# Rinoahu/SwiftOrtho

Measured on AMD Instinct MI355X. Metric: M query-aa/s scanned all-vs-all, higher is better.
Workload: dtype u8/int16/int32 (5-bit packed residues, packed 16-bit score-only DP, int32 traced DP); 1 GPU; BASELINE config 3: 100000 synthetic proteins x 300 aa self-search, seed 11111011111, aa9, -M 120000000, -c 50000 (2 chunks), -e 1e-5, -v 500; query_aa=30007201, rows=1618760

## Files before the change

swiftortho_amd/csrc/host.h:

```cpp
#pragma once
#include "common.h"
#include "kernels.h"
#include "seedhash.h"
#include "../../include/sohit.h"

#include <algorithm>
#include <array>
#include <atomic>
#include <chrono>
#include <cmath>
#include <cstring>
#include <functional>
#include <map>
#include <malloc.h>
#include <memory>
#include <mutex>
#include <thread>
#include <unordered_map>
#include <sys/stat.h>

inline double wall() { return std::chrono::duration<double>(std::chrono::steady_clock::now().time_since_epoch()).count(); }

extern double (*volatile p_pow)(double, double);
extern double (*volatile p_log)(double);
// ... 269 lines not shown
    u32 nq = 0;
    std::vector<u8> h_res;
    std::vector<u32> h_off;
    u32 maxqlen = 0;
    std::vector<u32> qid;
    std::vector<u8> qcls;
    u64 lay_gen = 0;
    i64 lay_lo = -1, lay_hi = -1;
    bool lay_classes = false;
    bool permuted = false;
    bool cls_sorted = true;
    u32 cls_start[QCLASSES_MAX + 1] = {0};
    u32 cls_maxq[QCLASSES_MAX] = {0};
    std::vector<u32> blkmax;
    u32 q_defer = 0;
    bool korder_async = false;
    bool korder_ready = false;
    u32 ksc_long = 0;
    DevBuf<u32> open_list;
    u32 n_open = 0;
    DevBuf<u8> kord_have;
    bool kord_have_clear = false;
    DevBuf<u32> d_qid, d_ocnt, d_ostart;
    SeqSet dev;
    DevBuf<u32> qbucket, korder, sbeg, scnt, pcnt, eff, nz, hoff, cidx;
    DevBuf<u32> sbeg2, scnt2, pcnt2;
    int bnd_ci = -1;
    DevBuf<int> ksc;
    DevBuf<u8> mark;
    DevBuf<u32> cs_hoff, cs_beg, blk_first, qseg, sel_idx;
    DevBuf<unsigned long long> qhits;
    DevBuf<u64> cs_kbase;
    DevBuf<u64> keys, keys2;
    DevBuf<u32> hits32, hits32s, bmat, bpart, bt0, btd, bext, bflag, bcnt, bccnt;
    DevBuf<u64> mlist;
    DevBuf<u32> flags, gidx, ghead;
    DevBuf<u64> p_qs, p_sd, p_ft, p_qs2, tmp64, q_qs, q_sd, q_ft;
    DevBuf<u32> shard;
    DevBuf<unsigned long long> stepshard;
    DevBuf<u32> pidx, pidx2, shead;
    DevBuf<u64> c_ft, c_ft2;
    DevBuf<u32> c_q, c_rec, order, order2;
    DevBuf<u32> counters;
    DevBuf<unsigned long long> ucount;
    DevBuf<u32> cand_q, cand_rec;
    std::vector<u32> chunk_base;
    DevBuf<u32> ccnt;
    DevBuf<unsigned long long> qcells;
    DevBuf<u32> tpos, spcnt, spoff, sidx, spec_trace, sel_a, sel_b;
    DevBuf<u64> gx;
    DevBuf<u32> gL, gR;
    DevBuf<u32> segfirst, st_state, rcnt, tcnt, roff, ridx, ridx2, ntile, roffc, rk_slot, order_tmp;
    DevBuf<u32> cqoff, prior, qtot, qcoff, fin_rec, perm, ntask, toff, sel, nout, ooff;
    DevBuf<AlnTask> tasks;
    DevBuf<AlnRes> ares;
    DevBuf<int> bits, outrec;
    DevBuf<u32> trace;
    DevBuf<u32> tr_units, tr_ofs;
    DevBuf<u32> tl_sorted, al_sorted;
    AlnChain aln;
};

#define QCLASSES 5
static_assert(QCLASSES <= QCLASSES_MAX, "Batch::cls_start");
inline u8 query_class(u32 len) { return len < 512 ? 0 : len < 1024 ? 1 : len < 2048 ? 2 : len < 4096 ? 3 : 4; }

// ... 278 lines not shown
```

swiftortho_amd/csrc/host_seed.hip:

```cpp
#include "host.h"

static void defer_long_class(so_ctx* c, Batch& b, u32 q_long) {
    b.korder_async = q_long < b.nq && b.cls_sorted && b.qcls[q_long] != b.qcls[0];
    if (!b.korder_async) return;
    b.q_defer = q_long;
    while (b.q_defer > 0 && b.qcls[b.q_defer - 1] == b.qcls[q_long]) --b.q_defer;
    HIP_CHECK(hipEventRecord(c->ev_side_go, c->st));
    HIP_CHECK(hipStreamWaitEvent(c->st_side, c->ev_side_go, 0));
}

void order_queries(so_ctx* c, Batch& b) {
    const u32 q_long = b.ksc_long;
    const size_t nres = b.h_off[b.nq];
    if (q_long < b.nq) b.gx.ensure(nres + 4), b.gL.ensure(nres + 4), b.gR.ensure(nres + 4);
    defer_long_class(c, b, q_long);
    launch_ksc_order(b.dev.d_scls.p, b.dev.d_off.p, b.nq, q_long, c->cfg.mink, c->d_b62c.p, b.gx.p, b.gL.p, b.gR.p, b.korder.p, c->st,
                     b.korder_async ? c->st_side : c->st);
    if (b.korder_async) HIP_CHECK(hipEventRecord(c->ev_korder, c->st_side));
    b.korder_ready = true;
}

void order_open_queries(so_ctx* c, Batch& b, const unsigned long long* qh) {
    u32 q_long = b.nq;
    for (u32 q = b.ksc_long; q < b.nq && q_long == b.nq; ++q)
// ... 531 lines not shown
                          c->ref.d_ug_store.p + U1_UG_PAD, c->ref.d_off.p + ch.seq_lo, c->d_b62c.p, b.bflag.p + 1, b.shard.p, b.p_qs.p, b.p_sd.p, b.p_ft.p, b.stepshard.p,
                          ug2 ? b.mlist.p : nullptr, b.bflag.p + 3, ugstat, c->st);
        if (ug2)
            launch_ungap2(c->ncu, b.mlist.p, b.bflag.p + 3, b.hits32s.p, b.bext.p, L, kl, klr, btab, U1_WAIT, b.dev.d_ug_store.p + U1_UG_PAD, b.dev.d_off.p,
                          c->ref.d_ug_store.p + U1_UG_PAD, c->ref.d_off.p + ch.seq_lo, c->d_b62c.p, b.bflag.p + 2, b.shard.p, b.p_qs.p, b.p_sd.p, b.p_ft.p, b.stepshard.p,
                          ugstat, c->st);
        else
            launch_ungap(w32 ? nullptr : b.keys2.p, Hv, kl, klr, btab, pmaxq >= gallop_min, ft_walk, b.dev.d_scls.p, b.dev.d_off.p, c->ref.d_scls4.p,
                         c->ref.d_off.p + ch.seq_lo, c->d_b62c.p, b.shard.p, shard_cap, b.p_qs.p, b.p_sd.p, b.p_ft.p, b.stepshard.p, c->st, w32 ? b.hits32s.p : nullptr,
                         b.bext.p, nb, &L, ug1, ugstat);
        bL = L;
        bL.R = (u32)(((u64)nseq_chunk + (1ull << wb) - 1) >> wb);
        bnb = bL.R * nqp;
        c->cnt.hits_bucketed += H;
        return true;
    };

    auto group_sorted = [&] {
    b.keys.ensure((size_t)H + 2), b.keys2.ensure((size_t)H + 2);
    const u32 nseg = qb - qa;
    const bool uq = tune().ungapq && tune().segsort && AS == 1 && compact && !ft_walk && UG_SHARDS == 1 && pmaxq <= ungapq_qcap() && nseg >= 256;
    if (uq || nseg >= 256) {
        b.qseg.ensure((size_t)b.nq + 4);
        launch_query_segments(b.hoff.p, b.dev.d_off.p, qa, qb, AS, H, b.qseg.p, c->st);
    }
    if (uq) {
        if (!c->ref.ug_valid) {
            const size_t nres = c->ref.res.size();
            c->ref.d_ug_store.ensure(nres + 2 * (size_t)U1_UG_PAD);
            launch_make_ug(c->ref.d_scls.p, c->ref.d_off.p, (u32)c->ref.N, nres, 8u, c->ref.d_ug_store.p + U1_UG_PAD, c->st);
            c->ref.ug_valid = true;
        }
        b.blk_first.ensure((size_t)nseg + 4), b.flags.ensure((size_t)nseg + 4);
        ProfTimer pt(c, &c->cnt.lookup_ms, &c->cnt.lookup_launches);
        launch_ungapq(c->ncu, b.qseg.p + qa, nseg, qa, b.blk_first.p, b.cs_hoff.p, b.cs_beg.p, b.cs_kbase.p, K, dk32, kl, klr, btab, b.dev.d_scls.p, b.dev.d_off.p,
                      c->ref.d_ug_store.p + U1_UG_PAD, c->ref.d_off.p + ch.seq_lo, c->d_b62c.p, b.bflag.p + 1, b.shard.p, b.p_qs.p, b.p_sd.p, b.p_ft.p, b.stepshard.p,
                      b.keys.p, b.keys2.p, b.flags.p, ugstat, c->st);
        pt.stop();
        if (c->profile) c->cnt.lookup_bytes += (i64)8 * (i64)H;
    } else {
    b.blk_first.ensure((size_t)lookup_num_blocks(H) + 2);
    launch_lookup_blockfirst(b.cs_hoff.p, K, H, b.blk_first.p, c->st);
    {
        ProfTimer pt(c, &c->cnt.lookup_ms, &c->cnt.lookup_launches);
        launch_lookup(b.cs_hoff.p, b.cs_beg.p, b.cs_kbase.p, b.blk_first.p, K, H, compact ? (const void*)dk32 : (const void*)ch.dkeys.p,
                      compact, c->ref.d_off.p + ch.seq_lo, kl, ch.maxslen, b.keys.p, c->st);
        pt.stop();
        if (c->profile) c->cnt.lookup_bytes += (i64)8 * (i64)H;
    }
    }
    t1 = wall();
    sc.lap("seed.compact_lookup");
    const int seg_mode = (int)tune().segsort;
    if (seg_mode && nseg >= 256) {
        ensure_sort_tmp(c, sort_keys_u64_seg_temp_bytes(H, nseg, kl.sh_diag, kl.sh_q));
        if (uq) sort_keys_u64_seg2(c->d_sort_tmp.p, c->d_sort_tmp.cap, b.keys.p, b.keys2.p, H, nseg, b.qseg.p + qa, b.flags.p, kl.sh_diag, kl.sh_q, c->st);
        else sort_keys_u64_seg(c->d_sort_tmp.p, c->d_sort_tmp.cap, b.keys.p, b.keys2.p, H, nseg, b.qseg.p + qa, kl.sh_diag, kl.sh_q, c->st);
    } else {
    ensure_sort_tmp(c, sort_keys_u64_temp_bytes(H, kl.total));
    sort_keys_u64(c->d_sort_tmp.p, c->d_sort_tmp.cap, b.keys.p, b.keys2.p, H, kl.sh_diag, kl.total, c->st);
    }
    sc.lap("group.sort_keys");
    launch_ungap(b.keys2.p, H, kl, klr, btab, pmaxq >= gallop_min, ft_walk, b.dev.d_scls.p, b.dev.d_off.p, c->ref.d_scls4.p, c->ref.d_off.p + ch.seq_lo,
                 c->d_b62c.p, b.shard.p, shard_cap, b.p_qs.p, b.p_sd.p, b.p_ft.p, b.stepshard.p, c->st, nullptr, nullptr, 0, nullptr, false, ugstat);
    };

    reset_pass_lists();
    if (!group_bucketed()) {
        bbest = false;
        group_sorted();
// ... 183 lines not shown
```

swiftortho_amd/csrc/k_ungapq.hip:

```cpp
#include "ungap1.h"

#define UQ_WAVES 16
#define UQ_RING 128
#define UQ_TBITS 12
#define UQ_QCAP 512
#define UQ_QSLOT (UQ_QCAP + 2 * U1_QPAD)
#define UQ_TILE 256
#define UQ_WAVE_BYTES (UQ_QSLOT + (1 << UQ_TBITS) / 4 + UQ_RING * 4 + UQ_RING * 4 + UQ_RING * 2 + UQ_TILE * 8)

__device__ __forceinline__ u32 bk_scan_max16(u32 x) {
    x = max(x, (u32)__builtin_amdgcn_update_dpp(0, (int)x, 0x111, 0xf, 0xf, true));
    x = max(x, (u32)__builtin_amdgcn_update_dpp(0, (int)x, 0x112, 0xf, 0xf, true));
    x = max(x, (u32)__builtin_amdgcn_update_dpp(0, (int)x, 0x114, 0xf, 0xf, true));
    x = max(x, (u32)__builtin_amdgcn_update_dpp(0, (int)x, 0x118, 0xf, 0xf, true));
    x = max(x, (u32)__builtin_amdgcn_update_dpp(0, (int)x, 0x142, 0xa, 0xf, false));
    x = max(x, (u32)__builtin_amdgcn_update_dpp(0, (int)x, 0x143, 0xc, 0xf, false));
    return x;
}

__device__ __forceinline__ u32 uq_slot(u32 g) { return (g * 2654435761u) >> (32 - UQ_TBITS); }

__global__ __launch_bounds__(256) void k_uq_first(const u32* __restrict__ qseg, u32 nqp, const u32* __restrict__ cs_hoff, u32 K, u32* __restrict__ qk) {
    const u32 q = blockIdx.x * 256u + threadIdx.x;
    if (q > nqp) return;
    const u32 x = qseg[q];
    u32 lo = 0, hi = K;
    while (lo < hi) {
        const u32 m = (lo + hi) >> 1;
        if (cs_hoff[m] < x) lo = m + 1;
        else hi = m;
    }
    qk[q] = lo;
}

template <bool BANDS, bool COUNT>
__global__ __launch_bounds__(64 * UQ_WAVES, 1) __attribute__((amdgpu_num_sgpr(96))) void k_ungapq(
    const u32* __restrict__ qseg , u32 nqp, u32 qa, const u32* __restrict__ qk, const u32* __restrict__ cs_hoff,
    const u32* __restrict__ cs_base, const u64* __restrict__ cs_kbase, const u32* __restrict__ dk32, int bp, int bd, int sh_q, int sh_qpos, int sh_diag, int diag_off, int rbs,
    int rsh_subj, int rsh_diag, int rdoff, const uint2* __restrict__ btab, u32 wait_n, const u8* __restrict__ q_scls, const u32* __restrict__ qoff,
    const u8* __restrict__ r_ug, const u32* __restrict__ roff, const signed char* __restrict__ b62g, u32* __restrict__ work_ctr, u32* __restrict__ shard_cnt,
    u64* __restrict__ p_qs, u64* __restrict__ p_sd, u64* __restrict__ p_ft, unsigned long long* __restrict__ group_count, u64* __restrict__ keys,
    u64* __restrict__ keys_sorted, u32* __restrict__ seg_end, unsigned long long* __restrict__ stat ) {
    constexpr int TSH = 3;
    constexpr u32 TBYTES = (u32)U1_ROWS << (8 + TSH);
    __shared__ __align__(16) unsigned char uq_smem[TBYTES + UQ_WAVES * UQ_WAVE_BYTES];
    const int lane = threadIdx.x & 63, w = threadIdx.x >> 6;
    for (u32 i = threadIdx.x; i < U1_ROWS * 32u * 32u; i += 64 * UQ_WAVES) {
        const u32 q = i >> 10, s = (i >> 5) & 31u, l = i & 31u;
        const int v = (q < SCLS_N && s < SCLS_N) ? (int)b62g[q * SCLS_N + s] : -100;
        *reinterpret_cast<short*>(uq_smem + ((q << 11) | (s << 6) | (l << 1))) = (short)v;
    }
    __syncthreads();
    unsigned char* wbase = uq_smem + TBYTES + (u32)w * UQ_WAVE_BYTES;
    u8* qslot = wbase;
    u32* tab = reinterpret_cast<u32*>(wbase + UQ_QSLOT);
    u32* ring_s = tab + (1 << UQ_TBITS) / 16;
    u32* ring_g = ring_s + UQ_RING;
    u16* ring_q = reinterpret_cast<u16*>(ring_g + UQ_RING);
    u32* mbase = reinterpret_cast<u32*>(ring_q + UQ_RING);
    u16* marks = reinterpret_cast<u16*>(mbase + UQ_TILE);
    u16* mqpos = marks + UQ_TILE;
    static_assert(UQ_TILE == 256, "tile_marks clears the marks with two words per lane");
    static_assert(U1_PCAP * 8 <= 7 * 64 && UQ_WAVES <= U1_ROWS, "pass buffer in a table row's tail");
    u64* s_pass = reinterpret_cast<u64*>(uq_smem + ((u32)w << 11) + 25 * 64);
    u16* s_passq = reinterpret_cast<u16*>(uq_smem + ((u32)w << 11) + 25 * 64 + U1_PCAP * 8);
    static_assert(U1_PCAP * 8 + U1_PCAP * 2 <= 7 * 64, "row tail");
    const unsigned long long lt = (1ull << lane) - 1ull;
    const u32 lanebase = (u32)(size_t)(__attribute__((address_space(3))) unsigned char*)uq_smem + ((u32)(lane & 31) << 1);
    const u32 pmask = (1u << bp) - 1u;
    const u32 dmask = (1u << bd) - 1u;
    u32 npb = 0, ngroups = 0;
    u32 ch_pos = 0, ch_end = 0;
    U1Track tr_unused;
    U1Count ct;
    ct.n = 0;
    ct.start();

    for (;;) {
        u32 qrel = 0;
        if (lane == 0) qrel = atomicAdd(work_ctr, 1u);
        qrel = (u32)__builtin_amdgcn_readfirstlane((int)qrel);
        if (qrel >= nqp) break;
        const u32 h0 = (u32)__builtin_amdgcn_readfirstlane((int)qseg[qrel]), h1 = (u32)__builtin_amdgcn_readfirstlane((int)qseg[qrel + 1]);
        if (h0 == h1) {
            if (lane == 0) seg_end[qrel] = h0;
            continue;
        }
        const u32 k0 = (u32)__builtin_amdgcn_readfirstlane((int)qk[qrel]), k1 = (u32)__builtin_amdgcn_readfirstlane((int)qk[qrel + 1]);
        const u32 gq = qa + qrel;
        const u32 qb0 = (u32)__builtin_amdgcn_readfirstlane((int)qoff[gq]);
        const int ql = (int)((u32)__builtin_amdgcn_readfirstlane((int)qoff[gq + 1]) - qb0);
        for (int i = lane * 16; i < UQ_QSLOT; i += 64 * 16) {
            const int p0 = i - U1_QPAD;
            uint4 v = make_uint4(0x18181818u, 0x18181818u, 0x18181818u, 0x18181818u);
            if (p0 >= 0 && p0 < ql) {
                v = u1_load16(q_scls + qb0 + (u32)p0);
                u32* d = reinterpret_cast<u32*>(&v);
#pragma unroll
                for (int k = 0; k < 4; ++k) {
                    const int nv = min(max(ql - p0 - 4 * k, 0), 4);
                    const u32 m = nv >= 4 ? 0xFFFFFFFFu : ((1u << (8 * nv)) - 1u);
                    d[k] = (d[k] & m) | (0x18181818u & ~m);
                }
                if (p0 == 0) d[0] = (d[0] & 0xFFFFFF00u) | 0x18u;
            }
            *reinterpret_cast<uint4*>(qslot + i) = v;
        }
        reinterpret_cast<uint4*>(tab)[lane] = make_uint4(0, 0, 0, 0);
        u1_wave_sync();
        const int qr_max = U1_QPAD + ql;
        const u64 kq = (u64)gq << sh_q;

        const u32 n = h1 - h0;
        u32 t_next = k0;
        u32 c_base = 0, c_qpos = 0;
        auto tile_marks = [&](u32 tb) {
            reinterpret_cast<u32*>(marks)[lane] = 0, reinterpret_cast<u32*>(marks)[64 + lane] = 0;
            u1_wave_sync();
            for (;;) {
                const u32 k = t_next + (u32)lane;
                u32 o = 0xFFFFFFFFu;
                if (k < k1) o = cs_hoff[k] - h0 - tb;
                const bool in = o < (u32)UQ_TILE;
                if (in) {
                    marks[o] = (u16)(o + 1u);
                    mbase[o] = cs_base[k] + h0;
                    mqpos[o] = (u16)((u32)(cs_kbase[k] >> sh_qpos) & pmask);
                }
                const u32 cnt = (u32)__popcll(__ballot(in));
                t_next += cnt;
                if (cnt < 64u) break;
            }
            u1_wave_sync();
        };
        auto gen_step = [&](u32 tb, u32 st, u32& c, u32& qpos, u32& o) -> bool {
            o = tb + 64u * st + (u32)lane;
            const u32 p1 = bk_scan_max16((u32)marks[64u * st + (u32)lane]);
            u32 base = c_base;
            qpos = c_qpos;
            if (p1) base = mbase[p1 - 1u], qpos = (u32)mqpos[p1 - 1u];
            c_base = (u32)__builtin_amdgcn_readlane((int)base, 63), c_qpos = (u32)__builtin_amdgcn_readlane((int)qpos, 63);
            c = 0xFFFFFFFFu;
            if (o >= n) return false;
            c = dk32[base + o];
            return (int)c >= 0;
        };
        for (u32 tb = 0; tb < n; tb += UQ_TILE) {
            tile_marks(tb);
            const u32 nst = (min(n - tb, (u32)UQ_TILE) + 63u) / 64u;
            for (u32 st = 0; st < nst; ++st) {
                u32 c, qpos, o;
                if (gen_step(tb, st, c, qpos, o)) {
                    const u32 t = uq_slot(c + qpos), sh = (t & 15u) * 2u;
                    const u32 old = atomicOr(&tab[t >> 4], 1u << sh);
                    if ((old >> sh) & 1u) atomicOr(&tab[t >> 4], 2u << sh);
                }
            }
        }
        u1_wave_sync();

        auto flush = [&]() {
            const u32 at = u1_reserve(npb, lane, ch_pos, ch_end, &shard_cnt[0], U1_CHUNK);
            if ((u32)lane < npb) {
                const u64 e = s_pass[lane];
                const u32 G = (u32)e, qp = (u32)s_passq[lane];
                u32 gsubj;
                int dlt;
                if (BANDS) {
                    const uint2 be = btab[G >> bd];
                    gsubj = be.x;
                    dlt = (int)(be.y - G);
                } else {
                    gsubj = G >> bd;
                    dlt = diag_off - (int)(G & dmask);
                }
                p_qs[at] = ((u64)gq << rbs) | gsubj;
                p_sd[at] = (e & 0xFFFFFFFF00000000ull) | (u64)(u32)dlt;
                p_ft[at] = ((u64)gsubj << rsh_subj) | ((u64)(u32)(rdoff - dlt) << rsh_diag) | ((u64)qp << sh_qpos);
            }
            npb = 0;
        };
        t_next = k0, c_base = 0, c_qpos = 0;
        u32 g_tb = 0, g_st = 0, g_nst = (min(n, (u32)UQ_TILE) + 63u) / 64u;
        tile_marks(0);
        bool more = true;
        u32 ns = 0;
        u32 rfront = 0, rback = 0;
        bool working = false;
        int qR = 0, qL = 0;
        i64 sR = 0, sL = 0;
        u32 hG = 0, hq = 0;
        pk16 S = {0, 0}, M = {0, 0};
        for (;;) {
            const unsigned long long idleb = __ballot(!working);
            if (idleb && ((u32)__popcll(idleb) >= wait_n || idleb == ~0ull)) {
                while (rback - rfront <= UQ_RING - 64u && more) {
                    u32 c, qpos, o;
                    const bool valid = gen_step(g_tb, g_st, c, qpos, o);
                    bool sing = false;
                    u32 G = 0;
                    if (valid) {
                        G = c + qpos;
                        const u32 t = uq_slot(G);
                        sing = ((tab[t >> 4] >> ((t & 15u) * 2u)) & 3u) == 1u;
                    }
                    const unsigned long long sb_ = __ballot(sing), kb_ = __ballot(valid && !sing);
                    if (valid && !sing) keys[h0 + ns + (u32)__popcll(kb_ & lt)] = kq + ((u64)qpos << sh_diag) + ((u64)qpos << sh_qpos) + ((u64)c << sh_diag);
                    ns += (u32)__popcll(kb_);
                    if (sing) {
                        u32 gsubj;
                        int dlt;
                        if (BANDS) {
                            const uint2 be = btab[G >> bd];
                            gsubj = be.x;
                            dlt = (int)(be.y - G);
                        } else {
                            gsubj = G >> bd;
                            dlt = diag_off - (int)(G & dmask);
                        }
                        const u32 slot = (rback + (u32)__popcll(sb_ & lt)) & (UQ_RING - 1);
                        ring_s[slot] = roff[gsubj] + (u32)((int)qpos + dlt);
                        ring_g[slot] = G;
                        ring_q[slot] = (u16)qpos;
                    }
                    rback += (u32)__popcll(sb_);
                    if (++g_st >= g_nst) {
                        g_st = 0, g_tb += UQ_TILE;
                        if (g_tb < n) {
                            g_nst = (min(n - g_tb, (u32)UQ_TILE) + 63u) / 64u;
                            tile_marks(g_tb);
                        } else {
                            more = false;
                        }
                    }
                }
                u1_wave_sync();
                const u32 avail = rback - rfront;
                if (!working) {
                    const u32 rk = (u32)__popcll(idleb & lt);
                    if (rk < avail) {
                        const u32 slot = (rfront + rk) & (UQ_RING - 1);
                        const u32 sa = ring_s[slot];
                        hG = ring_g[slot], hq = (u32)ring_q[slot];
                        qR = U1_QPAD + (int)hq, qL = qR - 16;
                        sR = (i64)sa, sL = (i64)sa - 16;
                        S = pk16{0, 0}, M = pk16{0, 0};
                        if (COUNT) ct.start();
                        working = true;
                    }
                }
                const u32 taken = min((u32)__popcll(idleb), avail);
                rfront += taken;
                ngroups += taken;
                u1_wave_sync();
            }
            if (!__ballot(working)) {
                if (!more && rback == rfront) break;
                continue;
            }
            bool fin = false;
            if (working) {
                const uint4 qr4 = u1_lds16(qslot, qR), ql4 = u1_lds16(qslot, qL);
                const uint4 sr4 = u1_load16(r_ug + sR), sl4 = u1_load16(r_ug + sL);
                const u32 msk = u1_step<TSH, false, COUNT>(qr4, ql4, sr4, sl4, lanebase, S, M, tr_unused, 0, ct);
                qR = min(qR + 16, qr_max), qL = max(qL - 16, 0);
                sR += 16, sL -= 16;
                fin = msk == 0xFFFFFFFFu;
            }
            {
                const int score = (int)M.x + (int)M.y;
                bool todo = fin && score >= MIN_UNGAP;
                for (;;) {
                    const unsigned long long pb = __ballot(todo);
                    if (!pb) break;
                    const u32 room = U1_PCAP - npb, rk = (u32)__popcll(pb & lt);
                    if (todo && rk < room) {
                        s_pass[npb + rk] = ((u64)(u32)score << 32) | hG;
                        s_passq[npb + rk] = (u16)hq;
                        todo = false;
                    }
                    npb += min((u32)__popcll(pb), room);
                    u1_wave_sync();
                    if (npb == U1_PCAP) {
                        flush();
                        u1_wave_sync();
                    }
                }
                if (fin) working = false;
            }
        }
        if (npb) {
            flush();
            u1_wave_sync();
        }
        if (lane == 0) seg_end[qrel] = h0 + ns;
        for (u32 i = h0 + ns + (u32)lane; i < h1; i += 64) keys_sorted[i] = ~0ull;
    }
    for (u32 i = ch_pos + (u32)lane; i < ch_end; i += 64) p_qs[i] = UG_REC_NONE, p_ft[i] = 0;
    if (lane == 0 && ngroups) atomicAdd(&group_count[0], (unsigned long long)ngroups);
    if (COUNT) {
        unsigned long long nst = ct.n;
#pragma unroll
        for (int o = 32; o > 0; o >>= 1) nst += __shfl_xor(nst, o);
        if (lane == 0) atomicAdd(&stat[0], nst), atomicAdd(&stat[1], (unsigned long long)ngroups);
    }
}

u32 ungapq_qcap() { return UQ_QCAP; }

void launch_ungapq(u32 ncu, const u32* qseg, u32 nqp, u32 qa, u32* qk, const u32* cs_hoff, const u32* cs_base, const u64* cs_kbase, u32 K, const u32* dk32,
                   const KeyLayout& kl, const KeyLayout& klr, const void* btab, const u8* q_scls, const u32* qoff, const u8* r_ug, const u32* roff, const signed char* b62g,
                   u32* work_ctr, u32* shard_cnt, u64* p_qs, u64* p_sd, u64* p_ft, unsigned long long* group_count, u64* keys, u64* keys_sorted, u32* seg_end,
                   unsigned long long* stat, hipStream_t st) {
    if (!nqp) return;
    hipLaunchKernelGGL(k_uq_first, dim3((nqp + 1 + 255) / 256), dim3(256), 0, st, qseg, nqp, cs_hoff, K, qk);
    static_assert(((size_t)U1_ROWS << 11) + (size_t)UQ_WAVES * UQ_WAVE_BYTES <= 160 * 1024, "LDS of a CU");
    const dim3 g(std::min<u32>(ncu, (nqp + UQ_WAVES - 1) / UQ_WAVES)), bl(64 * UQ_WAVES);
#define UQ_GO(B, CT)                                                                                                                                              \
    hipLaunchKernelGGL((k_ungapq<B, CT>), g, bl, 0, st, qseg, nqp, qa, qk, cs_hoff, cs_base, cs_kbase, dk32, kl.bp, kl.bd, kl.sh_q, kl.sh_qpos, kl.sh_diag, (int)kl.diag_off, klr.bs,  \
                       klr.sh_subj, klr.sh_diag, (int)klr.diag_off, (const uint2*)btab, U1_WAIT, q_scls, qoff, r_ug, roff, b62g, work_ctr, shard_cnt, p_qs, p_sd, p_ft,      \
                       group_count, keys, keys_sorted, seg_end, stat)
    if (stat) {
        if (btab) UQ_GO(true, true);
        else UQ_GO(false, true);
    } else if (btab) UQ_GO(true, false);
    else UQ_GO(false, false);
#undef UQ_GO
}
```

swiftortho_amd/csrc/kernels.h:

```cpp
#pragma once
#include "common.h"

struct HashLut;

size_t scan_u32_temp_elems(size_t n);
size_t effscan_temp_elems(size_t n);
const u32* effscan(const u8* mark, const u32* scnt, size_t n, u32* hoff, u32* cidx, u32* temp, hipStream_t st);
const u32* scan_u32(const u32* in, u32* out, size_t n, bool inclusive, u32* temp, hipStream_t st);
void fill_u32(u32* p, size_t n, u32 v, hipStream_t st);

size_t sort_keys_u64_temp_bytes(size_t n, int bits);
void sort_keys_u64(void* temp, size_t temp_bytes, const u64* in, u64* out, size_t n, int begin_bit, int end_bit, hipStream_t st);
void launch_query_segments(const u32* hoff, const u32* qoff, u32 qa, u32 qb, int AS, u32 H, u32* seg, hipStream_t st);
size_t sort_keys_u64_seg_temp_bytes(size_t n, u32 nseg, int begin_bit, int end_bit);
void sort_keys_u64_seg(void* temp, size_t temp_bytes, const u64* in, u64* out, size_t n, u32 nseg, const u32* seg, int begin_bit,
                       int end_bit, hipStream_t st);
void sort_keys_u64_seg2(void* temp, size_t temp_bytes, const u64* in, u64* out, size_t n, u32 nseg, const u32* seg_begin, const u32* seg_end, int begin_bit,
                        int end_bit, hipStream_t st);
void launch_stride_gather(const u32* src, u32 stride, u32 n, u32* dst, hipStream_t st);
size_t sort_pairs_u64_u32_temp_bytes(size_t n, int bits);
void sort_pairs_u64_u32(void* temp, size_t temp_bytes, const u64* kin, u64* kout, const u32* vin, u32* vout, size_t n, int bits,
                        hipStream_t st);
size_t sort_pairs_u64_u64_temp_bytes(size_t n, int bits);
void sort_pairs_u64_u64(void* temp, size_t temp_bytes, const u64* kin, u64* kout, const u64* vin, u64* vout, size_t n, int bits,
// ... 47 lines not shown
void launch_cap(const u32* korder, const u32* qoff, u32 q0, u32 nq , int mink, const u32* pcnt, i64 threshold, u8* mark,
                unsigned long long* qhits, const u32* list, u32 nlist, hipStream_t st);
void launch_effcnt(const u8* mark, const u32* scnt, int AS, u32 p_lo, u32 p_hi, u32* eff, u32* nz, hipStream_t st);
void launch_compact_seeds(const u8* mark, const u32* scnt, const u32* hoff, const u32* cidx, const u32* sbeg, const u32* q_pseq, const u32* qoff,
                          u32 p_lo, u32 p_hi, int AS, const KeyLayout& kl, u32* cs_hoff, u32* cs_beg, u64* cs_kbase, hipStream_t st);
u32 lookup_num_blocks(u32 H);
void launch_lookup_blockfirst(const u32* cs_hoff, u32 K, u32 H, u32* wave_first, hipStream_t st);
void launch_lookup(const u32* cs_hoff, const u32* cs_base, const u64* cs_kbase, const u32* wave_first, u32 K, u32 H,
                   const void* dkeys , bool compact, const u32* roff, const KeyLayout& kl, u32 maxslen,
                   u64* keys, hipStream_t st);

void launch_group_list(const u32* flags, const u32* gidx, u32 H, u32* ghead, hipStream_t st);
u32 ungap_shard_cap(u32 H);
void launch_ungap(const u64* keys, u32 H, const KeyLayout& kl, const KeyLayout& klr, const void* btab, bool gallop, bool ft_walk, const u8* q_scls, const u32* qoff,
                  const u8* r_scls, const u32* roff, const signed char* b62g, u32* shard_cnt, u32 shard_cap, u64* p_qs, u64* p_sd,
                  u64* p_ft, unsigned long long* group_count, hipStream_t st,
                  const u32* words = nullptr, const u32* bext = nullptr, u32 nb = 0, const BktLayout* L = nullptr,
                  bool skip_single = false ,
                  unsigned long long* stat = nullptr );

#define UG_REC_NONE 0xFFFFFFFFFFFFFFFFull
#define U1_QCAP 2048
#define U1_UG_PAD 4096
u32 ungap1_qcap();
size_t ungap1_list_slack(u32 ncu);
void launch_make_ug(const u8* scls, const u32* off, u32 nseq, size_t nres, u32 mul, u8* out, hipStream_t st);
size_t ungap1_mlist_cap(u32 H, u32 ncu);
#define U1_WAIT 4u
void launch_ungap1(u32 ncu, u32 pmaxq, const u32* words, const u32* bext, u32 nb, const BktLayout& L, const KeyLayout& kl, const KeyLayout& klr,
                   const void* btab, u32 wait_n, const u8* q_scls, const u32* qoff, const u8* r_ug, const u32* roff, const signed char* b62g, u32* work_ctr ,
                   u32* shard_cnt, u64* p_qs, u64* p_sd, u64* p_ft, unsigned long long* group_count, u64* mlist, u32* mlist_cnt,
                   unsigned long long* stat , hipStream_t st);
u32 ungapq_qcap();
void launch_ungapq(u32 ncu, const u32* qseg, u32 nqp, u32 qa, u32* qk, const u32* cs_hoff, const u32* cs_base, const u64* cs_kbase, u32 K, const u32* dk32,
                   const KeyLayout& kl, const KeyLayout& klr, const void* btab, const u8* q_scls, const u32* qoff, const u8* r_ug, const u32* roff, const signed char* b62g,
                   u32* work_ctr, u32* shard_cnt, u64* p_qs, u64* p_sd, u64* p_ft, unsigned long long* group_count, u64* keys, u64* keys_sorted, u32* seg_end,
                   unsigned long long* stat, hipStream_t st);
void launch_ungap2(u32 ncu, const u64* mlist, const u32* mlist_cnt, const u32* words, const u32* bext, const BktLayout& L, const KeyLayout& kl, const KeyLayout& klr,
                   const void* btab, u32 wait_n, const u8* q_ug, const u32* qoff, const u8* r_ug, const u32* roff, const signed char* b62g, u32* work_ctr ,
                   u32* shard_cnt, u64* p_qs, u64* p_sd, u64* p_ft, unsigned long long* group_count, unsigned long long* stat ,
                   hipStream_t st);
void launch_first_touch(bool walk, const u64* keys, u32 H, const KeyLayout& kl, int ft_bits_entry, int bsp, const u32* roff, u64* p_ft, u32 n,
                        hipStream_t st);
void launch_shard_scan(const u32* shard_cnt, u32* shard_off, hipStream_t st);
void launch_compact_shards(const u32* shard_cnt, u32* shard_off, u32 shard_cap, const u64* a0, const u64* a1, const u64* a2, u64* b0,
                           u64* b1, u64* b2, hipStream_t st);
void launch_seg_flags(const u64* sorted_qs, u32 n, u32* flags, u32* zero_word , hipStream_t st);
int cand_order_lds_max();
int cand_order_lds_key_bits();
void launch_qseg(const u64* sorted_qs, u32 n, const u32* gidx, const u32* total, int bs, u32 q0, u32 q1, u32* seg, u32* maxseg, hipStream_t st);
int q_best_max();
void launch_qrec_scatter(const u64* p_qs, const u64* p_sd, const u64* p_ft, const u32* rnk, u32 n, int bs, u32 qa, const u32* qoff, u32* o_q, u32* o_subj,
                         u64* o_sd, u64* o_ft, hipStream_t st);
void launch_q_best(const u32* qoff, u32 qa, u32 nqp, const u32* o_subj, const u64* o_sd, const u64* o_ft, u32 seq_lo, int bsp, u32* t_rec, u32* perm,
                   u32* qcnt, u32* fallback, hipStream_t st);
void launch_q_emit(const u32* qoff, u32 qa, u32 nqp, u32 nslots, const u32* o_q, const u32* qcnt, const u32* coff, const u32* perm, const u32* t_rec,
                   u32* out_q, u32* out_rec, hipStream_t st);
void launch_cand_order_lds(const u64* c_ft, const u32* c_rec, const u32* seg, u32 q0, u32 q1, u32 maxseg, int bsp, u32* out_q, u32* out_rec, u32* qcnt,
                           hipStream_t st);
void launch_best(const u64* sorted_qs, const u32* idx, const u32* shead, u32 nseg, u32 n, const u64* p_sd, const u64* p_ft,
                 u32 seq_lo, int bs, u64* c_ft, u32* c_q, u32* c_rec, hipStream_t st);
void launch_gather_u32_as_u64(const u32* src, const u32* idx, u32 n, u64* dst, hipStream_t st);
void launch_iota(u32* p, u32 n, hipStream_t st);
void launch_combine_q_ft(const u32* c_q, const u64* c_ft, u32 n, int ftbits, int bsp, u64* dst, hipStream_t st);
void launch_emit_cands(const u32* order, u32 n, const u64* sorted_key , int qshift ,
                       const u32* c_rec, u32* out_q, u32* out_rec, u32* qcnt, u32* seg_first, hipStream_t st);

#define TRACE_WORD(b, l) ((((u32)(b) >> 2) << 6) | ((u32)(l) << 2) | ((u32)(b) & 3u))
u32 align_trace_stride(int max_rows);
void launch_align(const AlnTask* tasks, const u32* ridx, u32 ntasks, const AlnSeqs& s, AlnRes* out, hipStream_t st);
// ... 92 lines not shown
```

Baseline: 673.0 M query-aa/s.

## Split ungapped query kernel into classification and extension kernels

The fused k_ungapq kernel is split in two. A small 4-wave classification kernel, sized for eight workgroups per CU, writes non-singleton seed keys and dumps singleton hits into global lone lists. A separate extension kernel reads those lists into its ring and runs the ungapped extension, with two workgroups per CU when stats are off. The aim is higher occupancy for the light hashing phase and less LDS per extension workgroup, at the cost of an extra global round trip for the singleton lists, a second launch, and extra buffer memory.

Measured after the change: 646.4 M query-aa/s. 3.9% lower.

```diff
diff --git a/swiftortho_amd/csrc/host.h b/swiftortho_amd/csrc/host.h
--- a/swiftortho_amd/csrc/host.h
+++ b/swiftortho_amd/csrc/host.h
@@ -325,6 +325,7 @@
     DevBuf<unsigned long long> qhits;
     DevBuf<u64> cs_kbase;
     DevBuf<u64> keys, keys2;
+    DevBuf<u32> lone, lone_n;
     DevBuf<u32> hits32, hits32s, bmat, bpart, bt0, btd, bext, bflag, bcnt, bccnt;
     DevBuf<u64> mlist;
     DevBuf<u32> flags, gidx, ghead;
diff --git a/swiftortho_amd/csrc/host_seed.hip b/swiftortho_amd/csrc/host_seed.hip
--- a/swiftortho_amd/csrc/host_seed.hip
+++ b/swiftortho_amd/csrc/host_seed.hip
@@ -587,10 +587,11 @@
             c->ref.ug_valid = true;
         }
         b.blk_first.ensure((size_t)nseg + 4), b.flags.ensure((size_t)nseg + 4);
+        b.lone.ensure(ungapq_list_words(H) + 2), b.lone_n.ensure((size_t)nseg + 4);
         ProfTimer pt(c, &c->cnt.lookup_ms, &c->cnt.lookup_launches);
-        launch_ungapq(c->ncu, b.qseg.p + qa, nseg, qa, b.blk_first.p, b.cs_hoff.p, b.cs_beg.p, b.cs_kbase.p, K, dk32, kl, klr, btab, b.dev.d_scls.p, b.dev.d_off.p,
+        launch_ungapq(c->ncu, b.qseg.p + qa, nseg, qa, b.blk_first.p, b.cs_hoff.p, b.cs_beg.p, b.cs_kbase.p, K, H, dk32, kl, klr, btab, b.dev.d_scls.p, b.dev.d_off.p,
                       c->ref.d_ug_store.p + U1_UG_PAD, c->ref.d_off.p + ch.seq_lo, c->d_b62c.p, b.bflag.p + 1, b.shard.p, b.p_qs.p, b.p_sd.p, b.p_ft.p, b.stepshard.p,
-                      b.keys.p, b.keys2.p, b.flags.p, ugstat, c->st);
+                      b.keys.p, b.keys2.p, b.flags.p, b.lone.p, b.lone_n.p, ugstat, c->st);
         pt.stop();
         if (c->profile) c->cnt.lookup_bytes += (i64)8 * (i64)H;
     } else {
diff --git a/swiftortho_amd/csrc/k_ungapq.hip b/swiftortho_amd/csrc/k_ungapq.hip
--- a/swiftortho_amd/csrc/k_ungapq.hip
+++ b/swiftortho_amd/csrc/k_ungapq.hip
@@ -1,12 +1,13 @@
 #include "ungap1.h"
 
-#define UQ_WAVES 16
 #define UQ_RING 128
 #define UQ_TBITS 12
 #define UQ_QCAP 512
 #define UQ_QSLOT (UQ_QCAP + 2 * U1_QPAD)
 #define UQ_TILE 256
-#define UQ_WAVE_BYTES (UQ_QSLOT + (1 << UQ_TBITS) / 4 + UQ_RING * 4 + UQ_RING * 4 + UQ_RING * 2 + UQ_TILE * 8)
+#define UQC_WAVES 4
+#define UQC_WAVE_BYTES ((1 << UQ_TBITS) / 4 + UQ_TILE * 8)
+#define UQE_WAVE_BYTES (UQ_QSLOT + UQ_RING * 4 + UQ_RING * 4 + UQ_RING * 2)
 
 __device__ __forceinline__ u32 bk_scan_max16(u32 x) {
     x = max(x, (u32)__builtin_amdgcn_update_dpp(0, (int)x, 0x111, 0xf, 0xf, true));
@@ -33,48 +34,23 @@
     qk[q] = lo;
 }
 
-template <bool BANDS, bool COUNT>
-__global__ __launch_bounds__(64 * UQ_WAVES, 1) __attribute__((amdgpu_num_sgpr(96))) void k_ungapq(
+template <bool BANDS>
+__global__ __launch_bounds__(64 * UQC_WAVES) __attribute__((amdgpu_waves_per_eu(8, 8))) __attribute__((amdgpu_num_sgpr(96))) void k_uq_class(
     const u32* __restrict__ qseg , u32 nqp, u32 qa, const u32* __restrict__ qk, const u32* __restrict__ cs_hoff,
-    const u32* __restrict__ cs_base, const u64* __restrict__ cs_kbase, const u32* __restrict__ dk32, int bp, int bd, int sh_q, int sh_qpos, int sh_diag, int diag_off, int rbs,
-    int rsh_subj, int rsh_diag, int rdoff, const uint2* __restrict__ btab, u32 wait_n, const u8* __restrict__ q_scls, const u32* __restrict__ qoff,
-    const u8* __restrict__ r_ug, const u32* __restrict__ roff, const signed char* __restrict__ b62g, u32* __restrict__ work_ctr, u32* __restrict__ shard_cnt,
-    u64* __restrict__ p_qs, u64* __restrict__ p_sd, u64* __restrict__ p_ft, unsigned long long* __restrict__ group_count, u64* __restrict__ keys,
-    u64* __restrict__ keys_sorted, u32* __restrict__ seg_end, unsigned long long* __restrict__ stat ) {
-    constexpr int TSH = 3;
-    constexpr u32 TBYTES = (u32)U1_ROWS << (8 + TSH);
-    __shared__ __align__(16) unsigned char uq_smem[TBYTES + UQ_WAVES * UQ_WAVE_BYTES];
+    const u32* __restrict__ cs_base, const u64* __restrict__ cs_kbase, const u32* __restrict__ dk32, int bp, int bd, int sh_q, int sh_qpos, int sh_diag, int diag_off,
+    const uint2* __restrict__ btab, const u32* __restrict__ roff, u32* __restrict__ work_ctr, u64* __restrict__ keys, u64* __restrict__ keys_sorted,
+    u32* __restrict__ seg_end, u32* __restrict__ lone_s, u32* __restrict__ lone_g, u16* __restrict__ lone_q, u32* __restrict__ lone_n) {
+    __shared__ __align__(16) unsigned char uq_smem[UQC_WAVES * UQC_WAVE_BYTES];
     const int lane = threadIdx.x & 63, w = threadIdx.x >> 6;
-    for (u32 i = threadIdx.x; i < U1_ROWS * 32u * 32u; i += 64 * UQ_WAVES) {
-        const u32 q = i >> 10, s = (i >> 5) & 31u, l = i & 31u;
-        const int v = (q < SCLS_N && s < SCLS_N) ? (int)b62g[q * SCLS_N + s] : -100;
-        *reinterpret_cast<short*>(uq_smem + ((q << 11) | (s << 6) | (l << 1))) = (short)v;
-    }
-    __syncthreads();
-    unsigned char* wbase = uq_smem + TBYTES + (u32)w * UQ_WAVE_BYTES;
-    u8* qslot = wbase;
-    u32* tab = reinterpret_cast<u32*>(wbase + UQ_QSLOT);
-    u32* ring_s = tab + (1 << UQ_TBITS) / 16;
-    u32* ring_g = ring_s + UQ_RING;
-    u16* ring_q = reinterpret_cast<u16*>(ring_g + UQ_RING);
-    u32* mbase = reinterpret_cast<u32*>(ring_q + UQ_RING);
+    unsigned char* wbase = uq_smem + (u32)w * UQC_WAVE_BYTES;
+    u32* tab = reinterpret_cast<u32*>(wbase);
+    u32* mbase = tab + (1 << UQ_TBITS) / 16;
     u16* marks = reinterpret_cast<u16*>(mbase + UQ_TILE);
     u16* mqpos = marks + UQ_TILE;
     static_assert(UQ_TILE == 256, "tile_marks clears the marks with two words per lane");
-    static_assert(U1_PCAP * 8 <= 7 * 64 && UQ_WAVES <= U1_ROWS, "pass buffer in a table row's tail");
-    u64* s_pass = reinterpret_cast<u64*>(uq_smem + ((u32)w << 11) + 25 * 64);
-    u16* s_passq = reinterpret_cast<u16*>(uq_smem + ((u32)w << 11) + 25 * 64 + U1_PCAP * 8);
-    static_assert(U1_PCAP * 8 + U1_PCAP * 2 <= 7 * 64, "row tail");
     const unsigned long long lt = (1ull << lane) - 1ull;
-    const u32 lanebase = (u32)(size_t)(__attribute__((address_space(3))) unsigned char*)uq_smem + ((u32)(lane & 31) << 1);
     const u32 pmask = (1u << bp) - 1u;
     const u32 dmask = (1u << bd) - 1u;
-    u32 npb = 0, ngroups = 0;
-    u32 ch_pos = 0, ch_end = 0;
-    U1Track tr_unused;
-    U1Count ct;
-    ct.n = 0;
-    ct.start();
 
     for (;;) {
         u32 qrel = 0;
@@ -83,32 +59,13 @@
         if (qrel >= nqp) break;
         const u32 h0 = (u32)__builtin_amdgcn_readfirstlane((int)qseg[qrel]), h1 = (u32)__builtin_amdgcn_readfirstlane((int)qseg[qrel + 1]);
         if (h0 == h1) {
-            if (lane == 0) seg_end[qrel] = h0;
+            if (lane == 0) seg_end[qrel] = h0, lone_n[qrel] = 0;
             continue;
         }
         const u32 k0 = (u32)__builtin_amdgcn_readfirstlane((int)qk[qrel]), k1 = (u32)__builtin_amdgcn_readfirstlane((int)qk[qrel + 1]);
         const u32 gq = qa + qrel;
-        const u32 qb0 = (u32)__builtin_amdgcn_readfirstlane((int)qoff[gq]);
-        const int ql = (int)((u32)__builtin_amdgcn_readfirstlane((int)qoff[gq + 1]) - qb0);
-        for (int i = lane * 16; i < UQ_QSLOT; i += 64 * 16) {
-            const int p0 = i - U1_QPAD;
-            uint4 v = make_uint4(0x18181818u, 0x18181818u, 0x18181818u, 0x18181818u);
-            if (p0 >= 0 && p0 < ql) {
-                v = u1_load16(q_scls + qb0 + (u32)p0);
-                u32* d = reinterpret_cast<u32*>(&v);
-#pragma unroll
-                for (int k = 0; k < 4; ++k) {
-                    const int nv = min(max(ql - p0 - 4 * k, 0), 4);
-                    const u32 m = nv >= 4 ? 0xFFFFFFFFu : ((1u << (8 * nv)) - 1u);
-                    d[k] = (d[k] & m) | (0x18181818u & ~m);
-                }
-                if (p0 == 0) d[0] = (d[0] & 0xFFFFFF00u) | 0x18u;
-            }
-            *reinterpret_cast<uint4*>(qslot + i) = v;
-        }
         reinterpret_cast<uint4*>(tab)[lane] = make_uint4(0, 0, 0, 0);
         u1_wave_sync();
-        const int qr_max = U1_QPAD + ql;
         const u64 kq = (u64)gq << sh_q;
 
         const u32 n = h1 - h0;
@@ -159,6 +116,110 @@
         }
         u1_wave_sync();
 
+        t_next = k0, c_base = 0, c_qpos = 0;
+        u32 ns = 0;
+        u32 nl = 0;
+        for (u32 tb = 0; tb < n; tb += UQ_TILE) {
+            tile_marks(tb);
+            const u32 nst = (min(n - tb, (u32)UQ_TILE) + 63u) / 64u;
+            for (u32 st = 0; st < nst; ++st) {
+                u32 c, qpos, o;
+                const bool valid = gen_step(tb, st, c, qpos, o);
+                bool sing = false;
+                u32 G = 0;
+                if (valid) {
+                    G = c + qpos;
+                    const u32 t = uq_slot(G);
+                    sing = ((tab[t >> 4] >> ((t & 15u) * 2u)) & 3u) == 1u;
+                }
+                const unsigned long long sb_ = __ballot(sing), kb_ = __ballot(valid && !sing);
+                if (valid && !sing) keys[h0 + ns + (u32)__popcll(kb_ & lt)] = kq + ((u64)qpos << sh_diag) + ((u64)qpos << sh_qpos) + ((u64)c << sh_diag);
+                ns += (u32)__popcll(kb_);
+                if (sing) {
+                    u32 gsubj;
+                    int dlt;
+                    if (BANDS) {
+                        const uint2 be = btab[G >> bd];
+                        gsubj = be.x;
+                        dlt = (int)(be.y - G);
+                    } else {
+                        gsubj = G >> bd;
+                        dlt = diag_off - (int)(G & dmask);
+                    }
+                    const u32 at = h0 + nl + (u32)__popcll(sb_ & lt);
+                    lone_s[at] = roff[gsubj] + (u32)((int)qpos + dlt);
+                    lone_g[at] = G;
+                    lone_q[at] = (u16)qpos;
+                }
+                nl += (u32)__popcll(sb_);
+            }
+        }
+        if (lane == 0) seg_end[qrel] = h0 + ns, lone_n[qrel] = nl;
+        for (u32 i = h0 + ns + (u32)lane; i < h1; i += 64) keys_sorted[i] = ~0ull;
+    }
+}
+
+template <bool BANDS, bool COUNT, int WGS>
+__global__ __launch_bounds__(64 * U1_WAVES, WGS) __attribute__((amdgpu_num_sgpr(80))) void k_uq_ext(
+    const u32* __restrict__ qseg, u32 nqp, u32 qa, const u32* __restrict__ lone_s, const u32* __restrict__ lone_g, const u16* __restrict__ lone_q,
+    const u32* __restrict__ lone_n, int bd, int sh_qpos, int diag_off, int rbs, int rsh_subj, int rsh_diag, int rdoff, const uint2* __restrict__ btab, u32 wait_n,
+    const u8* __restrict__ q_scls, const u32* __restrict__ qoff, const u8* __restrict__ r_ug, const signed char* __restrict__ b62g, u32* __restrict__ work_ctr,
+    u32* __restrict__ shard_cnt, u64* __restrict__ p_qs, u64* __restrict__ p_sd, u64* __restrict__ p_ft, unsigned long long* __restrict__ group_count,
+    unsigned long long* __restrict__ stat ) {
+    constexpr int TSH = 3;
+    constexpr u32 TBYTES = (u32)U1_ROWS << (8 + TSH);
+    __shared__ __align__(16) unsigned char uq_smem[TBYTES + U1_WAVES * UQE_WAVE_BYTES];
+    const int lane = threadIdx.x & 63, w = threadIdx.x >> 6;
+    u1_fill_table<TSH>(uq_smem, b62g);
+    __syncthreads();
+    unsigned char* wbase = uq_smem + TBYTES + (u32)w * UQE_WAVE_BYTES;
+    u8* qslot = wbase;
+    u32* ring_s = reinterpret_cast<u32*>(wbase + UQ_QSLOT);
+    u32* ring_g = ring_s + UQ_RING;
+    u16* ring_q = reinterpret_cast<u16*>(ring_g + UQ_RING);
+    static_assert(UQE_WAVE_BYTES % 16 == 0 && UQ_QSLOT % 16 == 0, "16-byte aligned query slots");
+    static_assert(U1_PCAP * 8 + U1_PCAP * 2 <= 7 * 64 && U1_WAVES <= U1_ROWS, "pass buffer in a table row's tail");
+    u64* s_pass = reinterpret_cast<u64*>(uq_smem + ((u32)w << 11) + 25 * 64);
+    u16* s_passq = reinterpret_cast<u16*>(uq_smem + ((u32)w << 11) + 25 * 64 + U1_PCAP * 8);
+    const unsigned long long lt = (1ull << lane) - 1ull;
+    const u32 lanebase = (u32)(size_t)(__attribute__((address_space(3))) unsigned char*)uq_smem + ((u32)(lane & 31) << 1);
+    const u32 dmask = (1u << bd) - 1u;
+    u32 npb = 0, ngroups = 0;
+    u32 ch_pos = 0, ch_end = 0;
+    U1Track tr_unused;
+    U1Count ct;
+    ct.n = 0;
+    ct.start();
+
+    for (;;) {
+        u32 qrel = 0;
+        if (lane == 0) qrel = atomicAdd(work_ctr, 1u);
+        qrel = (u32)__builtin_amdgcn_readfirstlane((int)qrel);
+        if (qrel >= nqp) break;
+        const u32 nl = (u32)__builtin_amdgcn_readfirstlane((int)lone_n[qrel]);
+        if (!nl) continue;
+        const u32 h0 = (u32)__builtin_amdgcn_readfirstlane((int)qseg[qrel]);
+        const u32 gq = qa + qrel;
+        const u32 qb0 = (u32)__builtin_amdgcn_readfirstlane((int)qoff[gq]);
+        const int ql = (int)((u32)__builtin_amdgcn_readfirstlane((int)qoff[gq + 1]) - qb0);
+        for (int i = lane * 16; i < UQ_QSLOT; i += 64 * 16) {
+            const int p0 = i - U1_QPAD;
+            uint4 v = make_uint4(0x18181818u, 0x18181818u, 0x18181818u, 0x18181818u);
+            if (p0 >= 0 && p0 < ql) {
+                v = u1_load16(q_scls + qb0 + (u32)p0);
+                u32* d = reinterpret_cast<u32*>(&v);
+#pragma unroll
+                for (int k = 0; k < 4; ++k) {
+                    const int nv = min(max(ql - p0 - 4 * k, 0), 4);
+                    const u32 m = nv >= 4 ? 0xFFFFFFFFu : ((1u << (8 * nv)) - 1u);
+                    d[k] = (d[k] & m) | (0x18181818u & ~m);
+                }
+                if (p0 == 0) d[0] = (d[0] & 0xFFFFFF00u) | 0x18u;
+            }
+            *reinterpret_cast<uint4*>(qslot + i) = v;
+        }
+        u1_wave_sync();
+        const int qr_max = U1_QPAD + ql;
         auto flush = [&]() {
             const u32 at = u1_reserve(npb, lane, ch_pos, ch_end, &shard_cnt[0], U1_CHUNK);
             if ((u32)lane < npb) {
@@ -180,11 +241,7 @@
             }
             npb = 0;
         };
-        t_next = k0, c_base = 0, c_qpos = 0;
-        u32 g_tb = 0, g_st = 0, g_nst = (min(n, (u32)UQ_TILE) + 63u) / 64u;
-        tile_marks(0);
-        bool more = true;
-        u32 ns = 0;
+        u32 cur = 0;
         u32 rfront = 0, rback = 0;
         bool working = false;
         int qR = 0, qL = 0;
@@ -194,45 +251,16 @@
         for (;;) {
             const unsigned long long idleb = __ballot(!working);
             if (idleb && ((u32)__popcll(idleb) >= wait_n || idleb == ~0ull)) {
-                while (rback - rfront <= UQ_RING - 64u && more) {
-                    u32 c, qpos, o;
-                    const bool valid = gen_step(g_tb, g_st, c, qpos, o);
-                    bool sing = false;
-                    u32 G = 0;
-                    if (valid) {
-                        G = c + qpos;
-                        const u32 t = uq_slot(G);
-                        sing = ((tab[t >> 4] >> ((t & 15u) * 2u)) & 3u) == 1u;
-                    }
-                    const unsigned long long sb_ = __ballot(sing), kb_ = __ballot(valid && !sing);
-                    if (valid && !sing) keys[h0 + ns + (u32)__popcll(kb_ & lt)] = kq + ((u64)qpos << sh_diag) + ((u64)qpos << sh_qpos) + ((u64)c << sh_diag);
-                    ns += (u32)__popcll(kb_);
-                    if (sing) {
-                        u32 gsubj;
-                        int dlt;
-                        if (BANDS) {
-                            const uint2 be = btab[G >> bd];
-                            gsubj = be.x;
-                            dlt = (int)(be.y - G);
-                        } else {
-                            gsubj = G >> bd;
-                            dlt = diag_off - (int)(G & dmask);
-                        }
-                        const u32 slot = (rback + (u32)__popcll(sb_ & lt)) & (UQ_RING - 1);
-                        ring_s[slot] = roff[gsubj] + (u32)((int)qpos + dlt);
-                        ring_g[slot] = G;
-                        ring_q[slot] = (u16)qpos;
-                    }
-                    rback += (u32)__popcll(sb_);
-                    if (++g_st >= g_nst) {
-                        g_st = 0, g_tb += UQ_TILE;
-                        if (g_tb < n) {
-                            g_nst = (min(n - g_tb, (u32)UQ_TILE) + 63u) / 64u;
-                            tile_marks(g_tb);
-                        } else {
-                            more = false;
-                        }
-                    }
+                while (rback - rfront <= UQ_RING - 64u && cur < nl) {
+                    const u32 i = cur + (u32)lane;
+                    if (i < nl) {
+                        const u32 slot = (rback + (u32)lane) & (UQ_RING - 1);
+                        ring_s[slot] = lone_s[h0 + i];
+                        ring_g[slot] = lone_g[h0 + i];
+                        ring_q[slot] = lone_q[h0 + i];
+                    }
+                    const u32 got = min(64u, nl - cur);
+                    rback += got, cur += got;
                 }
                 u1_wave_sync();
                 const u32 avail = rback - rfront;
@@ -255,7 +283,7 @@
                 u1_wave_sync();
             }
             if (!__ballot(working)) {
-                if (!more && rback == rfront) break;
+                if (cur >= nl && rback == rfront) break;
                 continue;
             }
             bool fin = false;
@@ -293,8 +321,6 @@
             flush();
             u1_wave_sync();
         }
-        if (lane == 0) seg_end[qrel] = h0 + ns;
-        for (u32 i = h0 + ns + (u32)lane; i < h1; i += 64) keys_sorted[i] = ~0ull;
     }
     for (u32 i = ch_pos + (u32)lane; i < ch_end; i += 64) p_qs[i] = UG_REC_NONE, p_ft[i] = 0;
     if (lane == 0 && ngroups) atomicAdd(&group_count[0], (unsigned long long)ngroups);
@@ -307,23 +333,37 @@
 }
 
 u32 ungapq_qcap() { return UQ_QCAP; }
-
-void launch_ungapq(u32 ncu, const u32* qseg, u32 nqp, u32 qa, u32* qk, const u32* cs_hoff, const u32* cs_base, const u64* cs_kbase, u32 K, const u32* dk32,
+size_t ungapq_list_words(u32 H) { return 2 * ((size_t)H + 2) + ((size_t)H + 2 + 1) / 2; }
+
+void launch_ungapq(u32 ncu, const u32* qseg, u32 nqp, u32 qa, u32* qk, const u32* cs_hoff, const u32* cs_base, const u64* cs_kbase, u32 K, u32 H, const u32* dk32,
                    const KeyLayout& kl, const KeyLayout& klr, const void* btab, const u8* q_scls, const u32* qoff, const u8* r_ug, const u32* roff, const signed char* b62g,
                    u32* work_ctr, u32* shard_cnt, u64* p_qs, u64* p_sd, u64* p_ft, unsigned long long* group_count, u64* keys, u64* keys_sorted, u32* seg_end,
-                   unsigned long long* stat, hipStream_t st) {
+                   u32* lone, u32* lone_n, unsigned long long* stat, hipStream_t st) {
     if (!nqp) return;
     hipLaunchKernelGGL(k_uq_first, dim3((nqp + 1 + 255) / 256), dim3(256), 0, st, qseg, nqp, cs_hoff, K, qk);
-    static_assert(((size_t)U1_ROWS << 11) + (size_t)UQ_WAVES * UQ_WAVE_BYTES <= 160 * 1024, "LDS of a CU");
-    const dim3 g(std::min<u32>(ncu, (nqp + UQ_WAVES - 1) / UQ_WAVES)), bl(64 * UQ_WAVES);
-#define UQ_GO(B, CT)                                                                                                                                              \
-    hipLaunchKernelGGL((k_ungapq<B, CT>), g, bl, 0, st, qseg, nqp, qa, qk, cs_hoff, cs_base, cs_kbase, dk32, kl.bp, kl.bd, kl.sh_q, kl.sh_qpos, kl.sh_diag, (int)kl.diag_off, klr.bs,  \
-                       klr.sh_subj, klr.sh_diag, (int)klr.diag_off, (const uint2*)btab, U1_WAIT, q_scls, qoff, r_ug, roff, b62g, work_ctr, shard_cnt, p_qs, p_sd, p_ft,      \
-                       group_count, keys, keys_sorted, seg_end, stat)
+    u32* lone_s = lone;
+    u32* lone_g = lone + ((size_t)H + 2);
+    u16* lone_q = reinterpret_cast<u16*>(lone + 2 * ((size_t)H + 2));
+    static_assert(8 * (size_t)UQC_WAVES * UQC_WAVE_BYTES <= 160 * 1024, "LDS of a CU: eight classification workgroups");
+    static_assert(2 * (((size_t)U1_ROWS << 11) + (size_t)U1_WAVES * UQE_WAVE_BYTES) <= 160 * 1024, "LDS of a CU: two extension workgroups");
+    {
+        const dim3 g(std::min<u32>(ncu * 8u, (nqp + UQC_WAVES - 1) / UQC_WAVES)), bl(64 * UQC_WAVES);
+#define UQC_GO(B)                                                                                                                                                    \
+    hipLaunchKernelGGL((k_uq_class<B>), g, bl, 0, st, qseg, nqp, qa, qk, cs_hoff, cs_base, cs_kbase, dk32, kl.bp, kl.bd, kl.sh_q, kl.sh_qpos, kl.sh_diag, (int)kl.diag_off, \
+                       (const uint2*)btab, roff, work_ctr, keys, keys_sorted, seg_end, lone_s, lone_g, lone_q, lone_n)
+        if (btab) UQC_GO(true);
+        else UQC_GO(false);
+#undef UQC_GO
+    }
+    const dim3 bl(64 * U1_WAVES);
+#define UQE_GO(B, CT, W)                                                                                                                                            \
+    hipLaunchKernelGGL((k_uq_ext<B, CT, W>), dim3(std::min<u32>(ncu * W, (nqp + U1_WAVES - 1) / U1_WAVES)), bl, 0, st, qseg, nqp, qa, lone_s, lone_g, lone_q, lone_n, kl.bd, \
+                       kl.sh_qpos, (int)kl.diag_off, klr.bs, klr.sh_subj, klr.sh_diag, (int)klr.diag_off, (const uint2*)btab, U1_WAIT, q_scls, qoff, r_ug, b62g,  \
+                       work_ctr + 1, shard_cnt, p_qs, p_sd, p_ft, group_count, stat)
     if (stat) {
-        if (btab) UQ_GO(true, true);
-        else UQ_GO(false, true);
-    } else if (btab) UQ_GO(true, false);
-    else UQ_GO(false, false);
-#undef UQ_GO
-}
+        if (btab) UQE_GO(true, true, 1);
+        else UQE_GO(false, true, 1);
+    } else if (btab) UQE_GO(true, false, 2);
+    else UQE_GO(false, false, 2);
+#undef UQE_GO
+}
diff --git a/swiftortho_amd/csrc/kernels.h b/swiftortho_amd/csrc/kernels.h
--- a/swiftortho_amd/csrc/kernels.h
+++ b/swiftortho_amd/csrc/kernels.h
@@ -103,10 +103,11 @@
                    u32* shard_cnt, u64* p_qs, u64* p_sd, u64* p_ft, unsigned long long* group_count, u64* mlist, u32* mlist_cnt,
                    unsigned long long* stat , hipStream_t st);
 u32 ungapq_qcap();
-void launch_ungapq(u32 ncu, const u32* qseg, u32 nqp, u32 qa, u32* qk, const u32* cs_hoff, const u32* cs_base, const u64* cs_kbase, u32 K, const u32* dk32,
+size_t ungapq_list_words(u32 H);
+void launch_ungapq(u32 ncu, const u32* qseg, u32 nqp, u32 qa, u32* qk, const u32* cs_hoff, const u32* cs_base, const u64* cs_kbase, u32 K, u32 H, const u32* dk32,
                    const KeyLayout& kl, const KeyLayout& klr, const void* btab, const u8* q_scls, const u32* qoff, const u8* r_ug, const u32* roff, const signed char* b62g,
-                   u32* work_ctr, u32* shard_cnt, u64* p_qs, u64* p_sd, u64* p_ft, unsigned long long* group_count, u64* keys, u64* keys_sorted, u32* seg_end,
-                   unsigned long long* stat, hipStream_t st);
+                   u32* work_ctr , u32* shard_cnt, u64* p_qs, u64* p_sd, u64* p_ft, unsigned long long* group_count, u64* keys, u64* keys_sorted,
+                   u32* seg_end, u32* lone, u32* lone_n, unsigned long long* stat, hipStream_t st);
 void launch_ungap2(u32 ncu, const u64* mlist, const u32* mlist_cnt, const u32* words, const u32* bext, const BktLayout& L, const KeyLayout& kl, const KeyLayout& klr,
                    const void* btab, u32 wait_n, const u8* q_ug, const u32* qoff, const u8* r_ug, const u32* roff, const signed char* b62g, u32* work_ctr ,
                    u32* shard_cnt, u64* p_qs, u64* p_sd, u64* p_ft, unsigned long long* group_count, unsigned long long* stat ,
```
